# JzHuai0108/sim3opt

Hardware: AMD Instinct MI355X
Metric: LM iterations/s (higher is better)
Workload: dtype f64

## Files before the change

sim3opt_amd/csrc/amg_kernels.hpp:

```cpp
#pragma once

__global__ __launch_bounds__(WG) void k_amg_adjoint(int nb, const int32_t* __restrict__ row2v,
                                                    const Sim3* __restrict__ states,
                                                    double* __restrict__ P) {
  for (int i = blockIdx.x * WG + threadIdx.x; i < nb; i += gridDim.x * WG) {
  const Sim3 S = load_sim3(states + row2v[i]);
  double R[9];
  sim3::R_from_quat(S.q, R);
  double A[49];
#pragma unroll
  for (int k = 0; k < 49; ++k) A[k] = 0.0;
  const double t0 = S.t[0], t1 = S.t[1], t2 = S.t[2];
#pragma unroll
  for (int c = 0; c < 3; ++c) {
    const double v0 = R[c], v1 = R[3 + c], v2 = R[6 + c];
    A[0 + 7 * c] = v0;
    A[1 + 7 * c] = v1;
    A[2 + 7 * c] = v2;
    A[3 + 7 * c] = t1 * v2 - t2 * v1;
    A[4 + 7 * c] = t2 * v0 - t0 * v2;
    A[5 + 7 * c] = t0 * v1 - t1 * v0;
    A[3 + 7 * (3 + c)] = S.s * v0;
    A[4 + 7 * (3 + c)] = S.s * v1;
    A[5 + 7 * (3 + c)] = S.s * v2;
  }
  A[3 + 42] = -t0;
  A[4 + 42] = -t1;
  A[5 + 42] = -t2;
  A[6 + 42] = 1.0;
  double* dst = P + (size_t)49 * i;
#pragma unroll
  for (int k = 0; k < 49; ++k) dst[k] = A[k];
  }
}

template <bool HASP>
__global__ __launch_bounds__(WG) void k_amg_galerkin(int cb0, int cb1, const int32_t* __restrict__ gptr,
                                                     const int32_t* __restrict__ gblk,
                                                     const int32_t* __restrict__ grow,
                                                     const int32_t* __restrict__ colidx_f,
                                                     const double* __restrict__ vals_f,
                                                     const double* __restrict__ P,
                                                     double* __restrict__ vals_c,
                                                     float* __restrict__ vals32_f) {
  const int lane = threadIdx.x & 63;
  const int cb = cb0 + __builtin_amdgcn_readfirstlane((int)(blockIdx.x * 4 + (threadIdx.x >> 6)));
  if (cb >= cb1) return;
  const int l49 = lane < 49 ? lane : lane - 49;
  const int r = l49 % 7, c = l49 / 7;
  double acc = 0.0;
  const int e0 = gptr[cb], e1 = gptr[cb + 1];
  for (int eb = e0; eb < e1; eb += 64) {
    const int n = e1 - eb < 64 ? e1 - eb : 64;
    const int le = lane < n ? lane : n - 1;
    const int kkv = gblk[eb + le];
    if (HASP) {
      const int giv = grow[eb + le];
      const int cjv = colidx_f[kkv];
      double av[2], pj[2][7], pi[2][7];
      int kk[2];
      auto load = [&](int u, int b) {
        kk[b] = __builtin_amdgcn_readlane(kkv, u);
        av[b] = vals_f[(size_t)49 * kk[b] + l49];
        const double* pjp = P + (size_t)49 * __builtin_amdgcn_readlane(cjv, u) + 7 * c;
        const double* pip = P + (size_t)49 * __builtin_amdgcn_readlane(giv, u) + 7 * r;
#pragma unroll
        for (int q = 0; q < 7; ++q) {
          pj[b][q] = pjp[q];
          pi[b][q] = pip[q];
        }
      };
      auto consume = [&](int b) {
        if (vals32_f && lane < 49) vals32_f[f32_pair_index(kk[b], lane)] = (float)av[b];
        double t = 0.0;
#pragma unroll
        for (int q = 0; q < 7; ++q) t += __shfl(av[b], r + 7 * q) * pj[b][q];
        double o = 0.0;
#pragma unroll
        for (int q = 0; q < 7; ++q) o += pi[b][q] * __shfl(t, q + 7 * c);
        acc += o;
      };
      for (int u = 0; u < n; ++u) {
        load(u, 0);
        consume(0);
      }
    } else {
      for (int u0 = 0; u0 < n; u0 += 4) {
        const int m = n - u0 < 4 ? n - u0 : 4;
        int kk[4];
        double av[4];
#pragma unroll
        for (int u = 0; u < 4; ++u)
          if (u < m) {
            kk[u] = __builtin_amdgcn_readlane(kkv, u0 + u);
            av[u] = vals_f[(size_t)49 * kk[u] + l49];
          }
#pragma unroll
        for (int u = 0; u < 4; ++u)
          if (u < m) {
            if (vals32_f && lane < 49) vals32_f[f32_pair_index(kk[u], lane)] = (float)av[u];
            acc += av[u];
          }
      }
    }
  }
  if (lane < 49) vals_c[(size_t)49 * cb + lane] = acc;
}

__global__ __launch_bounds__(WG) void k_amg_copydiag(int lo, int hi, const int32_t* __restrict__ rowptr,
                                                     const double* __restrict__ vals,
                                                     double* __restrict__ diagH) {
  for (int idx = 49 * lo + blockIdx.x * WG + threadIdx.x; idx < 49 * hi; idx += gridDim.x * WG)
    diagH[idx] = vals[(size_t)49 * rowptr[idx / 49] + idx % 49];
}

template <bool FIRST>
__global__ __launch_bounds__(WG) void k_amg_wsum(int nc, const int32_t* __restrict__ mptr,
                                                 const int32_t* __restrict__ mem,
                                                 const double* __restrict__ src,
                                                 double* __restrict__ Wc) {
  const int lane = threadIdx.x & 63;
  const int a = __builtin_amdgcn_readfirstlane((int)(blockIdx.x * 4 + (threadIdx.x >> 6)));
  if (a >= nc) return;
  const int l49 = lane < 49 ? lane : lane - 49;
  const int r = l49 % 7, c = l49 / 7;
  double acc = 0.0;
  for (int e = mptr[a]; e < mptr[a + 1]; ++e) {
    const double v = src[(size_t)49 * mem[e] + l49];
    if (FIRST) {
      double o = 0.0;
#pragma unroll
      for (int m = 0; m < 7; ++m) o += __shfl(v, m + 7 * r) * __shfl(v, m + 7 * c);
      acc += o;
    } else {
      acc += v;
    }
  }
  if (lane < 49) Wc[(size_t)49 * a + lane] = acc;
}


template <int K>
__global__ __launch_bounds__(WG) void k_amg_restrict(int a_lo, int nc, const int32_t* __restrict__ mptr,
                                                     const int32_t* __restrict__ mem,
                                                     const double* __restrict__ t_f,
                                                     double* __restrict__ r_c,
                                                     const double* __restrict__ Minv_c,
                                                     double* __restrict__ x_c, int64_t vs_f, int64_t vs_c,
                                                     int64_t ms_c) {
  const int lane = threadIdx.x & 63;
  const int wave = threadIdx.x >> 6;
  const int sub = lane / 7, rr = lane % 7, base = lane - rr;
  if (gridDim.y > 1) {
// ... 391 lines not shown
```

sim3opt_amd/csrc/engine_amg.hip:

```cpp
#include "engine_impl.hpp"

#include <cassert>

namespace sim3opt {

#include "spmv_kernel.hpp"
#include "amg_kernels.hpp"

int Engine::amg_init(const Structure& s, bool automatic, std::string& err) {
  (void)err;
  amg_omega = std::max(0.1, std::min(0.95, opt.amg_omega));
  amg_additive = opt.amg_additive != 0;
  {
    const bool partitioned = part_world() >= 2;
    int last = 0;
    for (int l = 1; l <= AMG_MAX_LEVELS; ++l) {
      const int o = l <= 4 ? opt.amg_cycle[l - 1] : 0;
      if (o >= 1 && o <= 3) last = o;
      amg_visits[l] = last > 0 ? last : (partitioned ? (l <= 1 ? 1 : 2) : (l <= 1 ? 2 : 3));
    }
    amg_visits[0] = 1;
  }
  amg_fp32 = opt.amg_fp32 != 0;
  adaptive_prec = opt.adaptive_prec != 0 && automatic;
// ... 101 lines not shown
  HIPCHK(mem.alloc(d_Ainv2, nc * nc, nullptr));
  HIPCHK(mem.alloc(d_piv, 2 * 28 * 28, nullptr));
#undef AMGCHK
  lvl_offs.assign(nl, std::vector<int64_t>());
  lvl_blk_offs.assign(nl, std::vector<int64_t>());
  for (int l = 1; l < nl; ++l) {
    amg[l].own_lo = 0; amg[l].own_hi = amg[l].nb;
    if (sharded(l - 1)) {
      const std::vector<int32_t> rb = H[l].row_begin.empty() ? std::vector<int32_t>{0, H[l].nb} : H[l].row_begin;
      amg[l].own_lo = rb[comm.rank];
      amg[l].own_hi = rb[comm.rank + 1];
      lvl_offs[l].resize(comm.world + 1);
      lvl_blk_offs[l].resize(comm.world + 1);
      for (int r = 0; r <= comm.world; ++r) {
        lvl_offs[l][r] = 7 * (int64_t)rb[r];
        lvl_blk_offs[l][r] = 49 * (int64_t)H[l].rowptr[rb[r]];
      }
    }
    amg[l].own_b0 = H[l].rowptr[amg[l].own_lo];
    amg[l].own_b1 = H[l].rowptr[amg[l].own_hi];
  }
  if (opt.verbose) {
    std::fprintf(stderr, "sim3opt: multigrid levels (rows/blocks):");
    for (const AmgLevel& L : amg) std::fprintf(stderr, " %d/%lld", L.nb, (long long)L.nnzb);
    if (comm.active()) std::fprintf(stderr, "; levels 0..%d partitioned over the ranks, the rest replicated", n_sharded - 1);
    std::fprintf(stderr, "; visits of levels 1, 2, 3: %d %d %d\n", amg_visits[1], amg_visits[2], amg_visits[3]);
  }
  cv_one = CycleView();
  cv_one.lv.resize(nl);
  for (int l = 0; l < nl; ++l) {
    cv_one.lv[l].Minv = amg[l].Minv;
    cv_one.lv[l].r = amg[l].r;
    cv_one.lv[l].x = amg[l].x;
    cv_one.lv[l].t = amg[l].t;
  }
  cv_one.sc = d_sc;
  cv_one.Ainv = d_Ainv;
  cv_one.rz_part = d_part_b;
  amg_host.clear();
  amg_host.shrink_to_fit();
  amg_stale = true;
  return SIM3OPT_OK;
}

int Engine::amg_setup(std::string& err) {
  const int nl = (int)amg.size();
  hipLaunchKernelGGL(k_amg_adjoint, dim3(grid_for(nb, WG)), dim3(WG), 0, stream, nb, d_row2v,
                     d_states, d_P);
  for (int l = 0; l + 1 < nl; ++l) {
    const AmgLevel& F = amg[l];
    AmgLevel& Cc = amg[l + 1];
    const int cb0 = (int)Cc.own_b0, cb1 = (int)Cc.own_b1;
    const int gg = std::max(1, (cb1 - cb0 + 3) / 4), gw = (Cc.nb + 3) / 4;
    if (l == 0)
      hipLaunchKernelGGL((k_amg_galerkin<true>), dim3(gg), dim3(WG), 0, stream, cb0, cb1, F.gptr,
                         F.gblk, F.grow, F.colidx, F.vals, d_P, Cc.vals, amg_fp32 ? F.vals32 : (float*)nullptr);
    else
      hipLaunchKernelGGL((k_amg_galerkin<false>), dim3(gg), dim3(WG), 0, stream, cb0, cb1, F.gptr,
                         F.gblk, F.grow, F.colidx, F.vals, (const double*)nullptr, Cc.vals,
                         amg_fp32 ? F.vals32 : (float*)nullptr);
    if (comm.active() && sharded(l) && !sharded(l + 1)) {
      int rc = comm.allgatherv(Cc.vals, lvl_blk_offs[l + 1], stream, err);
      if (rc) return rc;
    }
    if (l == 0)
      hipLaunchKernelGGL((k_amg_wsum<true>), dim3(gw), dim3(WG), 0, stream, Cc.nb, F.mptr, F.mem, d_P, Cc.W);
    else
      hipLaunchKernelGGL((k_amg_wsum<false>), dim3(gw), dim3(WG), 0, stream, Cc.nb, F.mptr, F.mem, F.W, Cc.W);
    hipLaunchKernelGGL(k_amg_copydiag, dim3(grid_for(49 * (int64_t)std::max(1, Cc.hi - Cc.lo), WG)), dim3(WG), 0, stream,
                       Cc.lo, Cc.hi, Cc.rowptr, Cc.vals, Cc.diagH);
  }
  if (amg_fp32)
    for (int l = nl - 1; l < nl; ++l) {
      const size_t cnt = (size_t)49 * (size_t)amg[l].nnzb;
      hipLaunchKernelGGL(k_to_f32, dim3(grid_for((int64_t)(cnt / 4), WG)), dim3(WG), 0, stream, cnt,
                         (const double*)amg[l].vals, amg[l].vals32);
    }
  HIPCHK(hipGetLastError());
  amg_stale = false;
  return SIM3OPT_OK;
}

void Engine::amg_prepare(double lambda) {
  const int nl = (int)amg.size();
  for (int l = 0; l < nl; ++l) {
    const AmgLevel& L = amg[l];
    const int lo = L.lo, hi = L.hi;
    jacobi(lo, hi, L.rowptr, L.vals, lambda, L.Minv, l == 0 && amg_additive ? 1.0 : amg_omega, L.diagH, L.W,
           l > 0 ? L.vals32 : (float*)nullptr);
  }
  dense_inverse(nullptr, d_Ainv, d_sc);
}

void Engine::dense_inverse(const double* diag64, double* Aout, DevScalars* sc) {
  const int nl = (int)amg.size();
  const AmgLevel& Lc = amg[nl - 1];
  const int nd = 7 * Lc.nb;
  auto pivot_rows = [&](int k0) { return nd - k0 >= amg_pivot ? amg_pivot : (nd - k0 >= 14 ? 14 : 7); };
  int nsteps = 0;
  for (int k0 = 0; k0 < nd; k0 += pivot_rows(k0)) ++nsteps;
  double *src = nsteps % 2 ? d_Ainv2 : Aout, *dst = nsteps % 2 ? Aout : d_Ainv2;
  (void)hipMemsetAsync(src, 0, sizeof(double) * (size_t)nd * nd, stream);
  hipLaunchKernelGGL(k_amg_dense_fill, dim3(grid_for(49 * Lc.nnzb, WG)), dim3(WG), 0, stream, Lc.nb,
                     Lc.rowptr, Lc.colidx, Lc.vals, src, diag64);
  double *pin = d_piv, *pout = d_piv + 28 * 28;
  switch (pivot_rows(0)) {
    case 28: hipLaunchKernelGGL((k_amg_dense_gj_first<28>), dim3(1), dim3(64), 0, stream, nd, (const double*)src, pin, sc); break;
    case 14: hipLaunchKernelGGL((k_amg_dense_gj_first<14>), dim3(1), dim3(64), 0, stream, nd, (const double*)src, pin, sc); break;
    default: hipLaunchKernelGGL((k_amg_dense_gj_first<7>), dim3(1), dim3(64), 0, stream, nd, (const double*)src, pin, sc);
  }
  const dim3 gt((nd + 63) / 64, (nd + 63) / 64 + 1);
  for (int k0 = 0; k0 < nd;) {
    const int pb = pivot_rows(k0), pbn = k0 + pb < nd ? pivot_rows(k0 + pb) : 0;
    if (pb == 28)
      hipLaunchKernelGGL((k_amg_dense_gj_step<28>), gt, dim3(WG), 0, stream, nd, k0, (const double*)src,
                         dst, (const double*)pin, pout, pbn, sc);
    else if (pb == 14)
      hipLaunchKernelGGL((k_amg_dense_gj_step<14>), gt, dim3(WG), 0, stream, nd, k0, (const double*)src,
                         dst, (const double*)pin, pout, pbn, sc);
    else
      hipLaunchKernelGGL((k_amg_dense_gj_step<7>), gt, dim3(WG), 0, stream, nd, k0, (const double*)src,
                         dst, (const double*)pin, pout, pbn, sc);
    k0 += pb;
    std::swap(src, dst);
    std::swap(pin, pout);
  }
}

void Engine::spmv_mode(const CycleView& V, int level, int mode, const double* v, double* out, const double* xc) {
  const AmgLevel& L = amg[level];
  const CycleLevel& B = V.lv[level];
  DevScalars* const sc = level == 0 ? V.sc : nullptr;
  double* const rz_part = level == 0 && mode == 2 && !amg_additive ? V.rz_part : nullptr;
  const BatchStrides bs{B.vs, B.ms, level + 1 < (int)amg.size() ? V.lv[level + 1].vs : 0, B.ms, V.part};
#define PASS(CHV, NTV, MODEV, VT, KV, DIAGV, SLICES, VALS)                                                           \
  hipLaunchKernelGGL((k_spmv_span<CHV, NTV, MODEV, VT, KV, DIAGV>), dim3(L.span_grid, SLICES), dim3(WG), 0, stream, \
                     L.nb, L.wrow, L.rowptr, L.colidx, (const VT*)(VALS), v, out, 0.0, rz_part, B.r,                 \
                     const_cast<double*>(xc), sc, (const double*)B.Minv, 1, (const int32_t*)L.agg, amg_over, bs,     \
                     (const float*)B.diag32)
#define PASS_FINE(CHV, VT, KV, VALS) \
  do { if (mode == 1) PASS(CHV, true, 1, VT, KV, false, 1, VALS); else PASS(CHV, true, 2, VT, KV, false, 1, VALS); } while (0)
#define PASS_COARSE(CHV, VT, KV, DIAGV, SLICES, VALS)                 \
  do {                                                                \
// ... 230 lines not shown
```

sim3opt_amd/csrc/engine_impl.hpp:

```cpp
#pragma once
#include <hip/hip_runtime.h>
#include <hip/hip_ext.h>

#include <algorithm>
#include <cfloat>
#include <chrono>
#include <cmath>
#include <cstdio>
#include <cstddef>
#include <cstdlib>
#include <cstring>

#include "amg.hpp"
#include "comm.hpp"
#include "devmem.hpp"
#include "direct_factor.hpp"
#include "engine.hpp"

namespace sim3opt {

using sim3::Sim3;

#ifndef SIM3OPT_COARSE_CH
#define SIM3OPT_COARSE_CH 8
// ... 319 lines not shown
  void spmv_mode(const CycleView& V, int level, int mode, const double* v, double* out, const double* xc = nullptr);

  void amg_restrict(const CycleView& V, int l, const double* t);
  void amg_prolong(const CycleView& V, int l, const double* xc, const double* xin, double* xout);

  double* amg_coarse(const CycleView& V, int l);
  double* amg_coarse_body(const CycleView& V, int l);
  void amg_exchange(int l, double* vec);

  double* amg_cycle(const CycleView& V, int l, double* cur, double* other);

  int amg_apply(std::string& err);

  int direct_init(const Structure& s, std::string& err);

  int direct_solve(double lambda, std::string& err);

  int debug_factor(int32_t context, double lambda, const double* vals, const double* b, bool with_solve,
                   bool with_selinv, double* Aperm, double* bp, double* L, double* Dinv, double* y, double* xp, double* x,
                   int32_t* fail, double* Z, int32_t* singular, int32_t* bord, int32_t* brow, std::string& err);

  BlockLdl marg_factor;
  std::vector<int32_t> mpos;
  std::string marg_refused;
  int marginal_init(std::string& err);
  int marginals(double lambda, int32_t n, const int32_t* row_a, const int32_t* row_b, double* cov,
                std::string& err);
  int cov_blocks(const char* who, bool any_pair, bool fixed_zero, double lambda, int32_t n, const int32_t* row_a,
                 const int32_t* row_b, double* cov, std::string& err);
  int64_t cov_stats[6] = {0, 0, 0, 0, 0, 0};
  int gate_edges(double lambda, int32_t n, const int32_t* v0, const int32_t* v1, const int32_t* row0,
                 const int32_t* row1, const Sim3* meas, const double* infoinv, double* e_out, double* S_out,
                 double* d2_out, std::string& err);
  DevArena cols_mem;
  double *c_g = nullptr, *c_y = nullptr, *c_r = nullptr, *c_d = nullptr;
  double* c_nrm = nullptr;
  int64_t c_vs = 0;
  int cols_alloc(std::string& err);
  void cols_release();
  int cols_batch_width() const {
    if (!use_amg || amg.empty() || comm.active() || !amg_fp32 || amg_additive) return 0;
    return opt.pcg_batch >= 1 ? std::min(opt.pcg_batch, KB) : KB;
  }
  int cols_solve(double lambda, int nsys, const double* g, const double* tol, bool setup, const double** x,
                 int32_t* iters, bool* failed, std::string& err);
  int cols_true_residuals(double lambda, int cnt, const int* sys, double* rel, std::string& err);
  int inverse_columns(double lambda, int32_t nvert, const int32_t* vertices, const int32_t* first,
                      const int32_t* blk_row, double* blocks, std::string& err);
  int cov_blocks_columns(const std::string& pre, bool fixed_zero, double lambda, int32_t n, const int32_t* row_a,
                         const int32_t* row_b, double* cov, std::string& err);
  int64_t col_counts[5] = {0, 0, 0, 0, 0};
  double col_res[2] = {0.0, 0.0};
  int32_t col_fail_vertex = -1;
  void jacobi(int lo, int hi, const int32_t* rowptr, double* vals, double lambda, double* Minv, double omega,
              const double* diagH, const double* W, float* vals32, DevScalars* sc = nullptr,
              double* diag64_out = nullptr, float* diag32_out = nullptr);
  void norms2(const double* r, const double* b, double* part_a, double* part_b, double* out2);
  void dense_inverse(const double* diag64, double* Aout, DevScalars* sc);

  int exchange_rows(double* vec, std::string& err) { return exchange_level(0, vec, err); }

  int chi2(double* out, std::string& err, hipEvent_t before_fetch = nullptr, int scale_parts = 0, int grid = 0);

  Sim3* d_ptab = nullptr;
  double ptab_delta = 0.0;
  sim3::Opts ptab_opts{0.0, -1, -1};

  int linearize(std::string& err);

  int spmv_chunk = 8, spmv_nt = 1;

  int spmv_grid() const { return span_grid; }

  void spmv_raw(double lambda, const double* v, double* q, const double* rvec, DevScalars* scp,
                hipEvent_t ev0 = nullptr, hipEvent_t ev1 = nullptr);

  int pcg_spmv(const PcgView& V, int live, const double* v, const double* rvec, bool timed, std::string& err);

  int agree_on_fail(std::string& err);

  int pcg(double lambda, int32_t* iters, double* rel_res, bool* ok, std::string& err);

  int pcg_attempt(double lambda, int prec, int32_t* iters, double* rel_res, bool* ok,
                  bool* chain_broke, std::string& err, int probe_budget = 0, bool* abandoned = nullptr,
                  const double* rhs = nullptr, double rel_tol = 0.0);
  int pcg_setup(PcgView& V, int prec, int nsetup, std::string& err);
  int pcg_run(PcgView& V, int prec, int nsetup, bool check_true, bool* setup_broke, std::string& err,
              int probe_budget = 0, bool* abandoned = nullptr);

  int diag_begin(PcgView& V, const double* lambda, int nrhs, const DevScalars* from, std::string& err);
  int amg_numbers(double lambda, std::string& err);
  int amg_level_readout(double lambda, int32_t level, int32_t* rowptr, int32_t* colidx, double* vals, float* vals32,
                        double* W, double* diagH, double* Minv, double* P, std::string& err);
  int amg_coarsest_inverse(double lambda, double* Ainv, std::string& err);
  int precond_apply(int prec, double lambda, int32_t nrhs, const double* r, double* z, std::string& err);
  int spmv_spans(int32_t* n_spans, int32_t* wrow, std::string& err);
  int operator_apply(int32_t nrhs, const double* lambda, const double* p, const double* rvec, double* q, double* pq,
                     double* rp, std::string& err);

  int iter_begin(sim3opt_iter_stats& T, double& chi, std::string& err);
  void iter_end(sim3opt_iter_stats& T, double chi, std::vector<sim3opt_iter_stats>& stats);
  bool direct_rejected() const;
  bool lin_dump = false;
  void apply_step(const double* x, bool push);
  void pop_states();

  int optimize(int32_t max_iters, std::vector<sim3opt_iter_stats>& stats, std::string& err);

  int optimize_gauss_newton(int32_t max_iters, std::vector<sim3opt_iter_stats>& stats, std::string& err);
// ... 24 lines not shown
```

sim3opt_amd/csrc/engine_pcg.hip:

```cpp
#include "engine_impl.hpp"

namespace sim3opt {

#include "spmv_kernel.hpp"
#include "pcg_kernels.hpp"

void Engine::jacobi(int lo, int hi, const int32_t* rowptr, double* vals, double lambda, double* Minv, double omega,
                    const double* diagH, const double* W, float* vals32, DevScalars* sc, double* diag64_out,
                    float* diag32_out) {
  hipLaunchKernelGGL(k_jacobi, dim3(std::max(1, (hi - lo + WG - 1) / WG)), dim3(WG), 0, stream, lo, hi, rowptr, vals,
                     lambda, Minv, sc ? sc : d_sc, omega, diagH, W, vals32, diag64_out, diag32_out);
}

void Engine::norms2(const double* r, const double* b, double* part_a, double* part_b, double* out2) {
  const int gn = grid_for(7 * (int64_t)(r1 - r0), WG);
  hipLaunchKernelGGL(k_norms2, dim3(gn), dim3(WG), 0, stream, 7 * r0, 7 * r1, r, b, part_a, part_b);
  hipLaunchKernelGGL(k_final_sum2<1>, dim3(1), dim3(WG), 0, stream, (const double*)part_a, (const double*)part_b, gn, 0,
                     out2, 0);
}

int Engine::level_part_init(int l, int32_t nb_l, const int32_t* rowptr_l, const int32_t* colidx_l,
                            const std::vector<int32_t>& row_begin_l, std::string& err) {
  LevelPart& lp = parts[l];
  lp.row_begin = row_begin_l;
  lp.lo = row_begin_l[comm.rank];
  lp.hi = row_begin_l[comm.rank + 1];
  lp.offs.resize(comm.world + 1);
  lp.blk_offs.resize(comm.world + 1);
  for (int r = 0; r <= comm.world; ++r) {
    lp.offs[r] = 7 * (int64_t)row_begin_l[r];
    lp.blk_offs[r] = 49 * (int64_t)rowptr_l[row_begin_l[r]];
  }
  if (!opt.halo_exchange || !comm.can_exchange()) return SIM3OPT_OK;
  std::vector<int32_t> srows, sseg, rrows, rseg;
  if (comm.world <= 1) {
    if (!comm.force) return SIM3OPT_OK;
    for (int32_t i = 0; i < std::min<int32_t>(nb_l, 64); ++i) srows.push_back(i);
    rrows = srows;
    sseg = {0, (int32_t)srows.size()};
    rseg = sseg;
    lp.self_test = true;
  } else {
    halo_plan(nb_l, rowptr_l, colidx_l, comm.world, row_begin_l.data(), comm.rank, srows, sseg, rrows, rseg);
  }
  lp.n_send = (int32_t)srows.size();
  lp.n_recv = (int32_t)rrows.size();
  {
    std::vector<int32_t> brows, bseg;
    boundary_rows(nb_l, rowptr_l, colidx_l, comm.world, row_begin_l.data(), brows, bseg);
    lp.neighbour = lp.self_test || 4 * (int64_t)brows.size() < 3 * (int64_t)nb_l;
  }
  if (opt.verbose)
    std::fprintf(stderr, "sim3opt: rank %d of %d, level %d: rows [%d, %d) of %d; sends %d rows, receives %d: %s\n",
                 comm.rank, comm.world, l, lp.lo, lp.hi, nb_l, lp.n_send, lp.n_recv,
                 lp.neighbour ? "neighbour exchange" : "whole-vector all-gather");
  if (!lp.neighbour) return SIM3OPT_OK;
  lp.send_offs.resize(comm.world + 1);
  lp.recv_offs.resize(comm.world + 1);
  for (int r = 0; r <= comm.world; ++r) {
    lp.send_offs[r] = 7 * (int64_t)sseg[r];
    lp.recv_offs[r] = 7 * (int64_t)rseg[r];
  }
  HIPCHK(upload(lp.d_send, srows));
  HIPCHK(upload(lp.d_recv, rrows));
// ... 528 lines not shown
    HIPCHK(batch_mem.alloc(B.Minv, (size_t)KB * B.ms, stream));
    if (l == 0) {
      B.r = b_r; B.x = b_z; B.t = b_az;
    } else {
      HIPCHK(batch_mem.alloc(B.r, (size_t)KB * B.vs, stream));
      HIPCHK(batch_mem.alloc(B.x, (size_t)KB * B.vs, stream));
      HIPCHK(batch_mem.alloc(B.t, (size_t)KB * B.vs, stream));
      HIPCHK(batch_mem.alloc(B.diag32, (size_t)KB * B.ms, stream));
    }
  }
  const size_t nc = (size_t)7 * amg[nl - 1].nb;
  b_as = (int64_t)(nc * nc);
  HIPCHK(batch_mem.alloc(b_Ainv, (size_t)KB * b_as, stream));
  HIPCHK(batch_mem.alloc(b_diag64, (size_t)KB * 49 * amg[nl - 1].nb, stream));
  HIPCHK(batch_mem.alloc(b_part_a, (size_t)KB * SPAN_GRID_MAX, stream));
  HIPCHK(batch_mem.alloc(b_part_b, (size_t)KB * SPAN_GRID_MAX, stream));
  HIPCHK(batch_mem.alloc(d_bsc, (size_t)KB, stream));
  HIPCHK(host_malloc((void**)&h_bsc, sizeof(DevScalars) * KB));
  V.sc = d_bsc;
  V.Ainv = b_Ainv;
  V.as = b_as;
  V.rz_part = b_part_b;
  V.part = SPAN_GRID_MAX;
  PcgView& P = pv_batch;
  P = PcgView();
  P.batch = true;
  P.nsc = KB;
  P.x = b_x; P.r = b_r; P.z = b_z; P.p = b_p; P.q = b_q; P.s = b_s; P.az = b_az;
  P.vs = b_vs;
  P.Minv = V.lv[0].Minv;
  P.ms = V.lv[0].ms;
  P.sc = d_bsc;
  P.h_sc = h_bsc;
  P.part_a = b_part_a;
  P.part_b = b_part_b;
  P.pstride = SPAN_GRID_MAX;
  P.cv = &cv_batch;
  batch_ready = true;
  return SIM3OPT_OK;
}

void Engine::batch_release() {
  batch_mem.release();
  if (h_bsc) host_free(h_bsc);
  h_bsc = nullptr;
  d_bsc = nullptr;
  cv_batch = CycleView();
  pv_batch = PcgView();
  batch_ready = false;
}

void Engine::batch_prepare(int nsetup) {
  const int nl = (int)amg.size();
  for (int s = 0; s < nsetup; ++s) {
    for (int l = 0; l < nl; ++l) {
      const AmgLevel& L = amg[l];
      const CycleLevel& B = cv_batch.lv[l];
      jacobi(0, L.nb, L.rowptr, L.vals, pv_batch.lam[s], B.Minv + (size_t)s * B.ms, amg_omega, L.diagH, L.W, nullptr,
             d_bsc + s, l == nl - 1 ? b_diag64 + (size_t)s * 49 * L.nb : nullptr,
             l > 0 ? B.diag32 + (size_t)s * B.ms : nullptr);
    }
    dense_inverse(b_diag64 + (size_t)s * 49 * amg[nl - 1].nb, b_Ainv + (size_t)s * b_as, d_bsc + s);
  }
}

int Engine::lm_trial_solve(int q, double lambda, double ni, const double** x, int32_t* iters, double* rel_res,
                           bool* ok, std::string& err) {
  TrialBatch& B = trial_batch;
  bool from_batch = q > 0 && B.next < B.n && B.lam[B.next] == lambda;
  if (!from_batch) {
    B.n = B.next = 0;
    const bool calm = B.prev_ok && !B.prev_capped && B.prev_pit > 0 && B.prev_pit <= 100;
    const int cap = q >= 1 && calm ? std::min(batch_capacity(), opt.max_trials - q) : 0;
    if (cap >= 2) {
      double gate = DBL_MAX;
      if (adaptive_prec && !trace_stale && mean_diag > 0.0) gate = bj_gate >= 0.0 ? bj_gate : 0.05 * mean_diag;
      int nsys = 0;
      double l = lambda, nu = ni;
      while (nsys < cap && l < gate && std::isfinite(l)) {
        B.lam[nsys++] = l;
        l *= nu;
        nu *= 2.0;
      }
      if (nsys >= 2) {
        bool usable = false;
        int rc = pcg_batch(B.lam, nsys, B.iters, B.rel, B.capped, &usable, err);
        if (rc) return rc;
        if (usable) {
          B.n = nsys;
          from_batch = true;
        }
      }
    }
  }
  if (from_batch) {
    const int s = B.next++;
    *x = b_x + (size_t)s * b_vs;
    *iters = B.iters[s];
    *rel_res = B.rel[s];
    *ok = true;
    last_capped = B.capped[s];
  } else {
    *x = d_x;
    int rc = pcg(lambda, iters, rel_res, ok, err);
    if (rc) return rc;
  }
  B.prev_ok = *ok;
  B.prev_capped = last_capped;
  B.prev_pit = *iters;
  return SIM3OPT_OK;
}

int SolverSnapshot::take(Engine& e, std::string& err) {
  eng = &e;
  HIPCHK(hipStreamSynchronize(e.stream));
  h_one = *e.h_sc;
// ... 217 lines not shown
```

sim3opt_amd/csrc/lm_kernels.hpp:

```cpp
#pragma once
__global__ __launch_bounds__(WG) void k_final_sum(const double* __restrict__ partials, int n,
                                                  double* __restrict__ out) {
  __shared__ double sh[4];
  const double s = sum_partials(partials, n, sh);
  if (threadIdx.x == 0) *out = s;
}

__global__ __launch_bounds__(WG) void k_final_trace_max(const double* __restrict__ trace_partials,
                                                        const double* __restrict__ max_partials, int n,
                                                        double* __restrict__ trace_out,
                                                        unsigned long long* __restrict__ maxdiag_bits) {
  __shared__ double sh[4];
  __shared__ double shm[4];
  const double s = sum_partials(trace_partials, n, sh);
  double m = 0.0;
  for (int i = threadIdx.x; i < n; i += WG) m = fmax(m, max_partials[i]);
#pragma unroll
  for (int off = 32; off > 0; off >>= 1) m = fmax(m, __shfl_xor(m, off));
  if ((threadIdx.x & 63) == 0) shm[threadIdx.x >> 6] = m;
  __syncthreads();
  if (threadIdx.x == 0) {
    *trace_out = s;
    m = fmax(fmax(shm[0], shm[1]), fmax(shm[2], shm[3]));
    *maxdiag_bits = (unsigned long long)__double_as_longlong(m);
// ... 334 lines not shown
    if (l < 14) {
      sim3::edge_jacobian_column(s_M[es], s_M[es] + sim3::JAC_SUMS, C, l, A.dof_mask, col);
    } else {
#pragma unroll
      for (int r = 0; r < 7; ++r) col[r] = e[r];
    }
#pragma unroll
    for (int r = 0; r < 7; ++r) s_J[es][l][r] = col[r];
  }
  linearize_gram_store<HAS_INFO, HAS_KERNEL, DUMP>(A, edge, valid, l, s_J[es], HAS_INFO ? s_O[es] : s_J[es], s_G[es], ai);
}

__global__ __launch_bounds__(WG) void k_edge_jacobians(EdgeArgs A, int dof_mask, double* __restrict__ e_out,
                                                      double* __restrict__ J_out) {
  for (int k = A.e_lo + blockIdx.x * WG + threadIdx.x; k < A.e_hi; k += gridDim.x * WG) {
    const Sim3 C = load_sim3(A.meas + k);
    const Sim3 S0 = load_sim3(A.states + A.ev0[k]);
    const Sim3 S1 = load_sim3(A.states + A.ev1[k]);
    double e[7], M[sim3::JAC_SUMS], X[13];
    sim3::edge_error(C, S0, S1, A.opts, e);
    sim3::left_jacobian_blocks(e, M);
    sim3::exp_of_residual(e, X);
#pragma unroll
    for (int r = 0; r < 7; ++r) e_out[(size_t)7 * k + r] = e[r];
    for (int c = 0; c < 14; ++c) {
      double col[7];
      sim3::edge_jacobian_column(M, X, C, c, dof_mask, col);
#pragma unroll
      for (int r = 0; r < 7; ++r) J_out[(size_t)98 * k + 14 * r + c] = col[r];
    }
  }
}

__global__ __launch_bounds__(WG) void k_diag_reduce(int r0, int r1,
                                                    const int32_t* __restrict__ incptr,
                                                    const int32_t* __restrict__ rowptr,
                                                    const double* __restrict__ scratch,
                                                    double* __restrict__ vals,
                                                    double* __restrict__ b, DevScalars* sc,
                                                    double* __restrict__ trace_partials,
                                                    double* __restrict__ max_partials) {
  __shared__ double sh[4];
  __shared__ double shm[4];
  const int lane = threadIdx.x & 63;
  const int wave = threadIdx.x >> 6;
  const int r = lane % 7, c = lane / 7;
  const int m = r < c ? r : c, M = r < c ? c : r;
  const int tsrc = lane < 49 ? (M * (M + 1)) / 2 + m : 0;
  const int bsrc = lane < 7 ? 28 + lane : 0;
  double dmax = 0.0, tr = 0.0;
  for (int row = r0 + blockIdx.x * 4 + wave; row < r1; row += gridDim.x * 4) {
    const int k0 = incptr[row], k1 = incptr[row + 1];
    double sum = 0.0;
    if (lane < 35)
      for (int k = k0; k < k1; ++k) sum += scratch[(size_t)35 * k + lane];
    const double v = __shfl(sum, tsrc);
    const double bv = __shfl(sum, bsrc);
    if (lane < 49) {
      vals[(size_t)49 * rowptr[row] + lane] = v;
      if (r == c) {
        dmax = fmax(dmax, fabs(v));
        tr += v;
      }
    }
    if (lane < 7) b[(size_t)7 * row + lane] = bv;
  }
#pragma unroll
  for (int off = 32; off > 0; off >>= 1) dmax = fmax(dmax, __shfl_xor(dmax, off));
  if (lane == 0) shm[wave] = dmax;
  const double ts = block_sum(tr, sh);
  if (threadIdx.x == 0) {
    trace_partials[blockIdx.x] = ts;
    max_partials[blockIdx.x] = fmax(fmax(shm[0], shm[1]), fmax(shm[2], shm[3]));
  }
}

__global__ __launch_bounds__(WG) void k_oplus(int nv, const int32_t* __restrict__ hidx,
                                              const double* __restrict__ x, Sim3* states,
                                              sim3::Opts opts, const DevScalars* sc, Sim3* backup,
                                              int fail_token) {
  const int v = blockIdx.x * WG + threadIdx.x;
  if (v >= nv) return;
  if (backup) {
    const double* s8 = reinterpret_cast<const double*>(states + v);
    double* b8 = reinterpret_cast<double*>(backup + v);
#pragma unroll
    for (int i = 0; i < 8; ++i) b8[i] = s8[i];
  }
  if (sc && sc->fail == fail_token) return;
  const int h = hidx[v];
  if (h < 0) return;
  double xi[7];
#pragma unroll
  for (int i = 0; i < 7; ++i) xi[i] = x[(size_t)7 * h + i];
  const Sim3 P = sim3::exp(xi, opts);
  const Sim3 S = sim3::mul(P, load_sim3(states + v));
  double* d = reinterpret_cast<double*>(states + v);
  d[0] = S.q[0]; d[1] = S.q[1]; d[2] = S.q[2]; d[3] = S.q[3];
  d[4] = S.t[0]; d[5] = S.t[1]; d[6] = S.t[2]; d[7] = S.s;
}

__global__ __launch_bounds__(WG) void k_copy_states(int nv, const Sim3* __restrict__ src, Sim3* __restrict__ dst) {
  const int i = blockIdx.x * WG + threadIdx.x;
  if (i < 8 * nv) reinterpret_cast<double*>(dst)[i] = reinterpret_cast<const double*>(src)[i];
}

__global__ __launch_bounds__(WG) void k_scale(int j0, int j1, const double* __restrict__ x,
                                              const double* __restrict__ b, double lambda,
// ... 17 lines not shown
```

sim3opt_amd/csrc/pcg_kernels.hpp:

```cpp
#pragma once
template <int K>
__global__ __launch_bounds__(WG) void k_final_sum2(const double* __restrict__ pa, const double* __restrict__ pb, int n,
                                                   int pstride, double* __restrict__ out2, int ostride) {
  __shared__ double sh[4];
#pragma unroll
  for (int s = 0; s < K; ++s) {
    const double a = sum_partials(pa + (size_t)s * pstride, n, sh);
    const double b = sum_partials(pb + (size_t)s * pstride, n, sh);
    if (threadIdx.x == 0) {
      out2[(size_t)s * ostride] = a;
      out2[(size_t)s * ostride + 1] = b;
    }
  }
}

__global__ void k_fail_to_double(DevScalars* sc) { sc->tmp_pq = sc->fail ? 1.0 : 0.0; }
__global__ void k_double_to_fail(DevScalars* sc) { if (sc->tmp_pq > 0.0) sc->fail = 1; }

__global__ __launch_bounds__(WG) void k_jacobi(int r0, int r1, const int32_t* __restrict__ rowptr,
                                               double* __restrict__ vals, double lambda,
                                               double* __restrict__ Minv, DevScalars* sc,
                                               double omega, const double* __restrict__ diagH,
                                               const double* __restrict__ W,
                                               float* __restrict__ vals32 = nullptr,
                                               double* __restrict__ diag64_out = nullptr,
                                               float* __restrict__ diag32_out = nullptr) {
  const int row = r0 + blockIdx.x * WG + threadIdx.x;
  if (row >= r1) return;
  double a[7][7];
  double* blk = vals + (size_t)49 * rowptr[row];
  const int64_t kd = rowptr[row];
  const double* src = diagH ? diagH + (size_t)49 * row : blk;
#pragma unroll
  for (int c = 0; c < 7; ++c)
#pragma unroll
    for (int r = 0; r < 7; ++r) a[r][c] = src[7 * c + r];
  if (W) {
    const double* w = W + (size_t)49 * row;
#pragma unroll
    for (int c = 0; c < 7; ++c)
#pragma unroll
      for (int r = 0; r < 7; ++r) {
        a[r][c] += lambda * w[7 * c + r];
        if (diag64_out || diag32_out) {
          if (diag64_out) diag64_out[(size_t)49 * row + 7 * c + r] = a[r][c];
          if (diag32_out) diag32_out[(size_t)49 * row + 7 * c + r] = (float)a[r][c];
        } else {
          blk[7 * c + r] = a[r][c];
          if (vals32) vals32[f32_pair_index(kd, 7 * c + r)] = (float)a[r][c];
        }
      }
  } else {
#pragma unroll
    for (int i = 0; i < 7; ++i) a[i][i] += lambda;
  }
  bool spd = true;
#pragma unroll
  for (int k = 0; k < 7; ++k) {
    if (!(a[k][k] > 0.0)) spd = false;
    const double d = 1.0 / a[k][k];
#pragma unroll
    for (int j = 0; j < 7; ++j)
      if (j != k) a[k][j] *= d;
#pragma unroll
    for (int i = 0; i < 7; ++i)
      if (i != k) {
        const double f = a[i][k];
#pragma unroll
        for (int j = 0; j < 7; ++j)
          if (j != k) a[i][j] -= f * a[k][j];
        a[i][k] = -f * d;
      }
    a[k][k] = d;
  }
  if (!spd) sc->fail = 1;
  double* dst = Minv + (size_t)49 * row;
#pragma unroll
  for (int r = 0; r < 7; ++r)
#pragma unroll
    for (int c = 0; c < 7; ++c) dst[7 * r + c] = omega * a[r][c];
}

template <int K, bool OWNB = false>
__global__ __launch_bounds__(WG) void k_pcg_init(int r0, int r1, const double* __restrict__ b,
                                                 const double* __restrict__ Minv, double* __restrict__ x,
                                                 double* __restrict__ r, double* __restrict__ z,
                                                 double* __restrict__ p, double* __restrict__ sv,
                                                 BatchStrides bs, int64_t bstride) {
  const int lane = threadIdx.x & 63;
  const int wave = threadIdx.x >> 6;
  const int sub = lane / 7, rr = lane % 7, base = lane - rr;
  for (int row0 = r0 + (blockIdx.x * 4 + wave) * 9; row0 < r1; row0 += gridDim.x * 36) {
    const int row = row0 + sub;
    const bool act = lane < 63 && row < r1;
    const size_t j = (size_t)7 * row + rr;
    double rv = act ? b[j] : 0.0;
#pragma unroll
    for (int s = 0; s < K; ++s) {
      const size_t o = (size_t)s * bs.vec;
      if (OWNB && s > 0) rv = act ? b[(size_t)s * bstride + j] : 0.0;
      if (act) {
        x[o + j] = 0.0;
        r[o + j] = rv;
        p[o + j] = 0.0;
        sv[o + j] = 0.0;
      }
      if (Minv) {
        double zv = 0.0;
#pragma unroll
        for (int cc = 0; cc < 7; ++cc) {
          const double rc = __shfl(rv, base + cc);
          if (act) zv += Minv[(size_t)s * bs.minv + (size_t)49 * row + 7 * rr + cc] * rc;
        }
        if (act) z[o + j] = zv;
      }
    }
  }
}

__global__ __launch_bounds__(64) void k_chain_factor(int r0, int r1, int seg,
                                                     const int32_t* __restrict__ rowptr,
                                                     const double* __restrict__ vals,
                                                     const int32_t* __restrict__ sub_first,
                                                     const int32_t* __restrict__ sub_cnt,
                                                     double lambda, double* __restrict__ Sinv,
                                                     double* __restrict__ Gm, DevScalars* sc) {
  const int sidx = blockIdx.x * 64 + threadIdx.x;
  const long long start = (long long)r0 + (long long)sidx * seg;
  if (start >= r1) return;
  const int row_end = (int)(start + seg < r1 ? start + seg : r1);
  double P[7][7];
  bool spd = true;
  for (int i = (int)start; i < row_end; ++i) {
// ... 274 lines not shown
```

Before: 50.98.

## Fuse per-level Jacobi launches, software-pipeline Galerkin loads, unroll incidence sums

Replaces the per-level and per-system k_jacobi launches with a single k_jacobi_levels kernel. It takes a struct of level descriptors and uses blockIdx.y over batched systems, which cuts launch count and host overhead. The level-0 Galerkin loop now prefetches the next fine block's value while computing the current one and uses sched barriers. The fp32 mirror write becomes a template flag, and the non-P path batches loads in groups of 16 and 8 for more memory-level parallelism. The incidence scatter-sum loop is unrolled by 8 and 4 with independent loads. The cost is a larger kernel-argument struct, a level-search loop in every block, and possible extra register pressure.

```diff
diff --git a/sim3opt_amd/csrc/amg_kernels.hpp b/sim3opt_amd/csrc/amg_kernels.hpp
--- a/sim3opt_amd/csrc/amg_kernels.hpp
+++ b/sim3opt_amd/csrc/amg_kernels.hpp
@@ -34,7 +34,24 @@
   }
 }
 
-template <bool HASP>
+template <int G>
+__device__ inline void galerkin_sum_group(int kkv, int u0, int lane, int l49, const double* __restrict__ vals_f,
+                                          float* __restrict__ vals32_f, double& acc) {
+  int kk[G];
+  double av[G];
+#pragma unroll
+  for (int u = 0; u < G; ++u) {
+    kk[u] = __builtin_amdgcn_readlane(kkv, u0 + u);
+    av[u] = vals_f[(size_t)49 * kk[u] + l49];
+  }
+#pragma unroll
+  for (int u = 0; u < G; ++u) {
+    if (vals32_f && lane < 49) vals32_f[f32_pair_index(kk[u], lane)] = (float)av[u];
+    acc += av[u];
+  }
+}
+
+template <bool HASP, bool F32>
 __global__ __launch_bounds__(WG) void k_amg_galerkin(int cb0, int cb1, const int32_t* __restrict__ gptr,
                                                      const int32_t* __restrict__ gblk,
                                                      const int32_t* __restrict__ grow,
@@ -57,35 +74,50 @@
     if (HASP) {
       const int giv = grow[eb + le];
       const int cjv = colidx_f[kkv];
-      double av[2], pj[2][7], pi[2][7];
-      int kk[2];
-      auto load = [&](int u, int b) {
-        kk[b] = __builtin_amdgcn_readlane(kkv, u);
-        av[b] = vals_f[(size_t)49 * kk[b] + l49];
-        const double* pjp = P + (size_t)49 * __builtin_amdgcn_readlane(cjv, u) + 7 * c;
-        const double* pip = P + (size_t)49 * __builtin_amdgcn_readlane(giv, u) + 7 * r;
+      auto load_a = [&](int u) {
+        return vals_f[(size_t)49 * __builtin_amdgcn_readlane(kkv, u < n ? u : n - 1) + l49];
+      };
+      double ahead = load_a(0);
+      __builtin_amdgcn_sched_barrier(0);
+      int kk = __builtin_amdgcn_readlane(kkv, 0);
+      int cj = __builtin_amdgcn_readlane(cjv, 0), gi = __builtin_amdgcn_readlane(giv, 0);
+      int u = 0;
+      do {
+        const double av = ahead;
+        const float a32 = (float)av;
+        const double* pjp = P + (size_t)49 * cj + 7 * c;
+        const double* pip = P + (size_t)49 * gi + 7 * r;
+        double pj[7], pi[7];
 #pragma unroll
         for (int q = 0; q < 7; ++q) {
-          pj[b][q] = pjp[q];
-          pi[b][q] = pip[q];
+          pj[q] = pjp[q];
+          pi[q] = pip[q];
         }
-      };
-      auto consume = [&](int b) {
-        if (vals32_f && lane < 49) vals32_f[f32_pair_index(kk[b], lane)] = (float)av[b];
+        __builtin_amdgcn_sched_barrier(0);
+        ahead = load_a(u + 1);
+        __builtin_amdgcn_sched_barrier(0);
         double t = 0.0;
 #pragma unroll
-        for (int q = 0; q < 7; ++q) t += __shfl(av[b], r + 7 * q) * pj[b][q];
+        for (int q = 0; q < 7; ++q) t += __shfl(av, r + 7 * q) * pj[q];
         double o = 0.0;
 #pragma unroll
-        for (int q = 0; q < 7; ++q) o += pi[b][q] * __shfl(t, q + 7 * c);
+        for (int q = 0; q < 7; ++q) o += pi[q] * __shfl(t, q + 7 * c);
         acc += o;
-      };
-      for (int u = 0; u < n; ++u) {
-        load(u, 0);
-        consume(0);
-      }
+        __builtin_amdgcn_sched_barrier(0);
+        if constexpr (F32) vals32_f[f32_pair_index(kk, l49)] = a32;
+        const int un = u + 1 < n ? u + 1 : n - 1;
+        kk = __builtin_amdgcn_readlane(kkv, un);
+        cj = __builtin_amdgcn_readlane(cjv, un);
+        gi = __builtin_amdgcn_readlane(giv, un);
+      } while (++u < n);
     } else {
-      for (int u0 = 0; u0 < n; u0 += 4) {
+      int u0 = 0;
+      for (; u0 + 16 <= n; u0 += 16) galerkin_sum_group<16>(kkv, u0, lane, l49, vals_f, F32 ? vals32_f : nullptr, acc);
+      if (u0 + 8 <= n) {
+        galerkin_sum_group<8>(kkv, u0, lane, l49, vals_f, F32 ? vals32_f : nullptr, acc);
+        u0 += 8;
+      }
+      for (; u0 < n; u0 += 4) {
         const int m = n - u0 < 4 ? n - u0 : 4;
         int kk[4];
         double av[4];
@@ -98,7 +130,7 @@
 #pragma unroll
         for (int u = 0; u < 4; ++u)
           if (u < m) {
-            if (vals32_f && lane < 49) vals32_f[f32_pair_index(kk[u], lane)] = (float)av[u];
+            if (F32 && lane < 49) vals32_f[f32_pair_index(kk[u], lane)] = (float)av[u];
             acc += av[u];
           }
       }
diff --git a/sim3opt_amd/csrc/engine_amg.hip b/sim3opt_amd/csrc/engine_amg.hip
--- a/sim3opt_amd/csrc/engine_amg.hip
+++ b/sim3opt_amd/csrc/engine_amg.hip
@@ -177,13 +177,14 @@
     AmgLevel& Cc = amg[l + 1];
     const int cb0 = (int)Cc.own_b0, cb1 = (int)Cc.own_b1;
     const int gg = std::max(1, (cb1 - cb0 + 3) / 4), gw = (Cc.nb + 3) / 4;
-    if (l == 0)
-      hipLaunchKernelGGL((k_amg_galerkin<true>), dim3(gg), dim3(WG), 0, stream, cb0, cb1, F.gptr,
-                         F.gblk, F.grow, F.colidx, F.vals, d_P, Cc.vals, amg_fp32 ? F.vals32 : (float*)nullptr);
-    else
-      hipLaunchKernelGGL((k_amg_galerkin<false>), dim3(gg), dim3(WG), 0, stream, cb0, cb1, F.gptr,
-                         F.gblk, F.grow, F.colidx, F.vals, (const double*)nullptr, Cc.vals,
-                         amg_fp32 ? F.vals32 : (float*)nullptr);
+#define GALERKIN(HASPV, F32V, PV, V32)                                                                         \
+  hipLaunchKernelGGL((k_amg_galerkin<HASPV, F32V>), dim3(gg), dim3(WG), 0, stream, cb0, cb1, F.gptr, F.gblk, F.grow, \
+                     F.colidx, F.vals, (const double*)(PV), Cc.vals, (float*)(V32))
+    if (l == 0 && amg_fp32) GALERKIN(true, true, d_P, F.vals32);
+    else if (l == 0) GALERKIN(true, false, d_P, nullptr);
+    else if (amg_fp32) GALERKIN(false, true, nullptr, F.vals32);
+    else GALERKIN(false, false, nullptr, nullptr);
+#undef GALERKIN
     if (comm.active() && sharded(l) && !sharded(l + 1)) {
       int rc = comm.allgatherv(Cc.vals, lvl_blk_offs[l + 1], stream, err);
       if (rc) return rc;
@@ -207,13 +208,7 @@
 }
 
 void Engine::amg_prepare(double lambda) {
-  const int nl = (int)amg.size();
-  for (int l = 0; l < nl; ++l) {
-    const AmgLevel& L = amg[l];
-    const int lo = L.lo, hi = L.hi;
-    jacobi(lo, hi, L.rowptr, L.vals, lambda, L.Minv, l == 0 && amg_additive ? 1.0 : amg_omega, L.diagH, L.W,
-           l > 0 ? L.vals32 : (float*)nullptr);
-  }
+  jacobi_levels(0, &lambda);
   dense_inverse(nullptr, d_Ainv, d_sc);
 }
 
diff --git a/sim3opt_amd/csrc/engine_impl.hpp b/sim3opt_amd/csrc/engine_impl.hpp
--- a/sim3opt_amd/csrc/engine_impl.hpp
+++ b/sim3opt_amd/csrc/engine_impl.hpp
@@ -395,9 +395,7 @@
   int64_t col_counts[5] = {0, 0, 0, 0, 0};
   double col_res[2] = {0.0, 0.0};
   int32_t col_fail_vertex = -1;
-  void jacobi(int lo, int hi, const int32_t* rowptr, double* vals, double lambda, double* Minv, double omega,
-              const double* diagH, const double* W, float* vals32, DevScalars* sc = nullptr,
-              double* diag64_out = nullptr, float* diag32_out = nullptr);
+  void jacobi_levels(int nsys, const double* lam);
   void norms2(const double* r, const double* b, double* part_a, double* part_b, double* out2);
   void dense_inverse(const double* diag64, double* Aout, DevScalars* sc);
 
diff --git a/sim3opt_amd/csrc/engine_pcg.hip b/sim3opt_amd/csrc/engine_pcg.hip
--- a/sim3opt_amd/csrc/engine_pcg.hip
+++ b/sim3opt_amd/csrc/engine_pcg.hip
@@ -5,11 +5,40 @@
 #include "spmv_kernel.hpp"
 #include "pcg_kernels.hpp"
 
-void Engine::jacobi(int lo, int hi, const int32_t* rowptr, double* vals, double lambda, double* Minv, double omega,
-                    const double* diagH, const double* W, float* vals32, DevScalars* sc, double* diag64_out,
-                    float* diag32_out) {
-  hipLaunchKernelGGL(k_jacobi, dim3(std::max(1, (hi - lo + WG - 1) / WG)), dim3(WG), 0, stream, lo, hi, rowptr, vals,
-                     lambda, Minv, sc ? sc : d_sc, omega, diagH, W, vals32, diag64_out, diag32_out);
+void Engine::jacobi_levels(int nsys, const double* lam) {
+  const int nl = (int)amg.size();
+  const bool batch = nsys > 0;
+  JacobiLevels A;
+  std::memset(&A, 0, sizeof(A));
+  A.nl = nl;
+  int wg = 0;
+  for (int l = 0; l < nl; ++l) {
+    const AmgLevel& L = amg[l];
+    JacobiLevel& J = A.lv[l];
+    J.lo = batch ? 0 : L.lo;
+    J.hi = batch ? L.nb : L.hi;
+    J.rowptr = L.rowptr;
+    J.vals = L.vals;
+    J.diagH = L.diagH;
+    J.W = L.W;
+    if (batch) {
+      const CycleLevel& B = cv_batch.lv[l];
+      J.Minv = B.Minv;
+      J.ms = B.ms;
+      J.omega = amg_omega;
+      J.diag64_out = l == nl - 1 ? b_diag64 : nullptr;
+      J.diag32_out = l > 0 ? B.diag32 : nullptr;
+    } else {
+      J.Minv = L.Minv;
+      J.omega = l == 0 && amg_additive ? 1.0 : amg_omega;
+      J.vals32 = l > 0 ? L.vals32 : nullptr;
+    }
+    wg += (J.hi - J.lo + WG - 1) / WG;
+    A.wg_end[l] = wg;
+  }
+  for (int s = 0; s < KB; ++s) A.lambda[s] = lam[std::min(s, std::max(nsys, 1) - 1)];
+  hipLaunchKernelGGL(k_jacobi_levels, dim3(std::max(1, wg), std::max(nsys, 1)), dim3(WG), 0, stream, A,
+                     batch ? d_bsc : d_sc);
 }
 
 void Engine::norms2(const double* r, const double* b, double* part_a, double* part_b, double* out2) {
@@ -644,16 +673,10 @@
 
 void Engine::batch_prepare(int nsetup) {
   const int nl = (int)amg.size();
-  for (int s = 0; s < nsetup; ++s) {
-    for (int l = 0; l < nl; ++l) {
-      const AmgLevel& L = amg[l];
-      const CycleLevel& B = cv_batch.lv[l];
-      jacobi(0, L.nb, L.rowptr, L.vals, pv_batch.lam[s], B.Minv + (size_t)s * B.ms, amg_omega, L.diagH, L.W, nullptr,
-             d_bsc + s, l == nl - 1 ? b_diag64 + (size_t)s * 49 * L.nb : nullptr,
-             l > 0 ? B.diag32 + (size_t)s * B.ms : nullptr);
-    }
+  if (nsetup <= 0) return;
+  jacobi_levels(nsetup, pv_batch.lam);
+  for (int s = 0; s < nsetup; ++s)
     dense_inverse(b_diag64 + (size_t)s * 49 * amg[nl - 1].nb, b_Ainv + (size_t)s * b_as, d_bsc + s);
-  }
 }
 
 int Engine::lm_trial_solve(int q, double lambda, double ni, const double** x, int32_t* iters, double* rel_res,
diff --git a/sim3opt_amd/csrc/lm_kernels.hpp b/sim3opt_amd/csrc/lm_kernels.hpp
--- a/sim3opt_amd/csrc/lm_kernels.hpp
+++ b/sim3opt_amd/csrc/lm_kernels.hpp
@@ -410,8 +410,34 @@
   for (int row = r0 + blockIdx.x * 4 + wave; row < r1; row += gridDim.x * 4) {
     const int k0 = incptr[row], k1 = incptr[row + 1];
     double sum = 0.0;
-    if (lane < 35)
-      for (int k = k0; k < k1; ++k) sum += scratch[(size_t)35 * k + lane];
+    if (lane < 35) {
+      const double* sp = scratch + (size_t)35 * k0 + lane;
+      int k = k0;
+      for (; k + 8 <= k1; k += 8, sp += 8 * 35) {
+        double s[8];
+#pragma unroll
+        for (int q = 0; q < 8; ++q) s[q] = sp[35 * q];
+#pragma unroll
+        for (int q = 0; q < 8; ++q) sum += s[q];
+      }
+      if (k + 4 <= k1) {
+        double s[4];
+#pragma unroll
+        for (int q = 0; q < 4; ++q) s[q] = sp[35 * q];
+#pragma unroll
+        for (int q = 0; q < 4; ++q) sum += s[q];
+        k += 4;
+        sp += 4 * 35;
+      }
+      const int m = k1 - k;
+      double s[3];
+#pragma unroll
+      for (int q = 0; q < 3; ++q)
+        if (q < m) s[q] = sp[35 * q];
+#pragma unroll
+      for (int q = 0; q < 3; ++q)
+        if (q < m) sum += s[q];
+    }
     const double v = __shfl(sum, tsrc);
     const double bv = __shfl(sum, bsrc);
     if (lane < 49) {
diff --git a/sim3opt_amd/csrc/pcg_kernels.hpp b/sim3opt_amd/csrc/pcg_kernels.hpp
--- a/sim3opt_amd/csrc/pcg_kernels.hpp
+++ b/sim3opt_amd/csrc/pcg_kernels.hpp
@@ -17,16 +17,11 @@
 __global__ void k_fail_to_double(DevScalars* sc) { sc->tmp_pq = sc->fail ? 1.0 : 0.0; }
 __global__ void k_double_to_fail(DevScalars* sc) { if (sc->tmp_pq > 0.0) sc->fail = 1; }
 
-__global__ __launch_bounds__(WG) void k_jacobi(int r0, int r1, const int32_t* __restrict__ rowptr,
-                                               double* __restrict__ vals, double lambda,
-                                               double* __restrict__ Minv, DevScalars* sc,
-                                               double omega, const double* __restrict__ diagH,
-                                               const double* __restrict__ W,
-                                               float* __restrict__ vals32 = nullptr,
-                                               double* __restrict__ diag64_out = nullptr,
-                                               float* __restrict__ diag32_out = nullptr) {
-  const int row = r0 + blockIdx.x * WG + threadIdx.x;
-  if (row >= r1) return;
+__device__ inline void jacobi_row(int row, const int32_t* __restrict__ rowptr, double* __restrict__ vals,
+                                  double lambda, double* __restrict__ Minv, DevScalars* sc, double omega,
+                                  const double* __restrict__ diagH, const double* __restrict__ W,
+                                  float* __restrict__ vals32, double* __restrict__ diag64_out,
+                                  float* __restrict__ diag32_out) {
   double a[7][7];
   double* blk = vals + (size_t)49 * rowptr[row];
   const int64_t kd = rowptr[row];
@@ -79,6 +74,46 @@
   for (int r = 0; r < 7; ++r)
 #pragma unroll
     for (int c = 0; c < 7; ++c) dst[7 * r + c] = omega * a[r][c];
+}
+
+__global__ __launch_bounds__(WG) void k_jacobi(int r0, int r1, const int32_t* __restrict__ rowptr,
+                                               double* __restrict__ vals, double lambda,
+                                               double* __restrict__ Minv, DevScalars* sc,
+                                               double omega, const double* __restrict__ diagH,
+                                               const double* __restrict__ W) {
+  const int row = r0 + blockIdx.x * WG + threadIdx.x;
+  if (row >= r1) return;
+  jacobi_row(row, rowptr, vals, lambda, Minv, sc, omega, diagH, W, nullptr, nullptr, nullptr);
+}
+
+struct JacobiLevel {
+  int32_t lo, hi;
+  const int32_t* rowptr;
+  double* vals;
+  double* Minv;
+  const double* diagH;
+  const double* W;
+  float* vals32;
+  double* diag64_out;
+  float* diag32_out;
+  double omega;
+  int64_t ms;
+};
+struct JacobiLevels {
+  int32_t nl;
+  int32_t wg_end[AMG_MAX_LEVELS];
+  JacobiLevel lv[AMG_MAX_LEVELS];
+  double lambda[KB];
+};
+__global__ __launch_bounds__(WG) void k_jacobi_levels(const JacobiLevels A, DevScalars* sc) {
+  int l = 0;
+  while (l + 1 < A.nl && (int)blockIdx.x >= A.wg_end[l]) ++l;
+  const JacobiLevel& L = A.lv[l];
+  const int row = L.lo + ((int)blockIdx.x - (l ? A.wg_end[l - 1] : 0)) * WG + (int)threadIdx.x;
+  if (row >= L.hi) return;
+  const size_t s = blockIdx.y, so = s * (size_t)L.ms;
+  jacobi_row(row, L.rowptr, L.vals, A.lambda[s], L.Minv + so, sc + s, L.omega, L.diagH, L.W, L.vals32,
+             L.diag64_out ? L.diag64_out + so : nullptr, L.diag32_out ? L.diag32_out + so : nullptr);
 }
 
 template <int K, bool OWNB = false>
```

After: 51.30 (median of 2 runs). About the same (+0.6%).
